# gnns4hri/3D_multi_pose_estimator

Hardware: AMD Instinct MI355X
Metric: frames/sec (5-view Panoptic, 4 persons) at 1/2/4/8 GPUs; MPJPE vs ref (higher is better)
Workload: dtype f32

## Files before the change

3d_multi_pose_estimator_amd/csrc/api.hip:

```cpp
#include <cmath>
#include <cstdarg>
#include <new>
#include <cstdio>
#include <cstdlib>
#include <cstring>

#include "mpe_internal.h"

using namespace mpe;

namespace {

int fail(mpe_ctx *ctx, int code, const char *fmt, ...) {
    char buf[512];
    va_list ap;
    va_start(ap, fmt);
    vsnprintf(buf, sizeof buf, fmt, ap);
    va_end(ap);
    if (ctx) ctx->err = buf;
    return code;
}

#define HIPCHK(ctx, expr)                                                                     \
    do {                                                                                      \
// ... 361 lines not shown
    const int V = ctx->cfg.n_cameras, J = ctx->cfg.n_joints, npj = ctx->cfg.numbers_per_joint;
    if (ctx->mlp[0].in_dim != V * J * npj)
        return fail(ctx, MPE_ERR_INVALID, "MLP input width %d != V*J*numbers_per_joint = %d", ctx->mlp[0].in_dim,
                    V * J * npj);
    int widest = 0;
    for (int l = 0; l < ctx->mlp_layers; ++l) {
        if (l > 0 && ctx->mlp[l].in_dim != ctx->mlp[l - 1].out_dim)
            return fail(ctx, MPE_ERR_INVALID, "MLP layer %d input width mismatch", l);
        widest = widest > ctx->mlp[l].out_dim ? widest : ctx->mlp[l].out_dim;
    }
    ctx->mlp_ld_in = round_up(ctx->mlp[0].in_dim, 128);
    ctx->mlp_ld_hidden = round_up(widest, 128);
    const size_t rows = (size_t)ctx->cfg.max_frames * ctx->cfg.max_persons_per_frame;
    int rc;
    if ((rc = dev_alloc(ctx, &ctx->mlp_rows, rows * ctx->mlp_ld_in))) return rc;
    for (int i = 0; i < 2; ++i)
        if ((rc = dev_alloc(ctx, &ctx->mlp_act[i], rows * ctx->mlp_ld_hidden))) return rc;
    ctx->mlp_ws_ready = true;
    return MPE_OK;
}

enum GatInput {
    GAT_IN_IMPLICIT,
    GAT_IN_DENSE0,
    GAT_IN_ACT
};

int gat_layer_linear(mpe_ctx *ctx, hipStream_t s, const mpe_batch *b, int l, GatInput in, AggArgs *a, int *n_rows_ft2) {
    GatLayer &g = ctx->gat[l];
    const int V = ctx->cfg.n_cameras, J = ctx->cfg.n_joints;
    const int n_nodes = b->n_heads + b->n_edge_nodes;
    const bool red = ctx->gat_reduced;
    const bool half_rows = red || ctx->gat_attn_fp16;
    const int ld_ft = half_rows ? 2 * ctx->act_ld : ctx->act_ld;
    int rc;
    const AttnCoef coef{g.attn_l, g.attn_r, ctx->a12, g.heads, g.out_dim};
    const bool no_epi = getenv("MPE_NO_COEF_EPILOGUE") != nullptr;
    const AttnCoef *cp = no_epi ? nullptr : &coef;
    bool done = false;
    if (in == GAT_IN_DENSE0) {
        if ((rc = gat_linear(ctx, s, ctx->xdense, ctx->feat_ld, g.fc1, ctx->hdense, ctx->feat_ld, n_nodes, nullptr,
                             true, ctx->gat_alpha, false)))
            return rc;
        if ((rc = gat_linear(ctx, s, ctx->hdense, ctx->feat_ld, g.fc2, ctx->act[2], ld_ft, n_nodes, nullptr, false,
                             0.f, half_rows, nullptr, nullptr, -1.0, cp, &done)))
            return rc;
        a->ft2 = ctx->act[2];
        *n_rows_ft2 = n_nodes;
    } else if (in == GAT_IN_IMPLICIT) {
        if (ctx->l0_grouped && !red && linear_uses_tile_kernel(b->n_heads, g.in_dim)) {
            GemmProf gp(ctx, s, 2.0 * b->n_heads * (double)g.in_dim * (J * 10), 0, 0);
            HIPCHK(ctx, launch_linear_grouped(s, ctx->xc, ctx->l0_ld, ctx->l0_w, ctx->l0_ld,
                                              (long)weight_rows(g.in_dim) * ctx->l0_ld, ctx->l0_b, ctx->h0, ctx->feat_ld,
                                              b->n_heads, ctx->cam_count, V, ctx->cam_list, ctx->cfg.max_heads, g.in_dim,
                                              ctx->l0_ld, true, ctx->gat_alpha, ctx->gat_acc64));
        } else if (ctx->l0_grouped) {
            const double flop_each = 2.0 * b->n_heads * (double)g.in_dim * (J * 10) / V;
            for (int c = 0; c < V; ++c)
                if ((rc = gat_linear(ctx, s, ctx->xc, ctx->l0_ld, ctx->l0_fc1[c], ctx->h0, ctx->feat_ld, b->n_heads,
                                     ctx->cam_count + c, true, ctx->gat_alpha, false,
                                     ctx->cam_list + (size_t)c * ctx->cfg.max_heads,
                                     ctx->cam_list + (size_t)c * ctx->cfg.max_heads, flop_each)))
                    return rc;
        } else if ((rc = gat_linear(ctx, s, ctx->x0, ctx->feat_ld, g.fc1, ctx->h0, ctx->feat_ld, b->n_heads, nullptr,
                                    true, ctx->gat_alpha, false)))
            return rc;
        if ((rc = gat_linear(ctx, s, ctx->h0, ctx->feat_ld, g.fc2, ctx->act[1], ld_ft, b->n_heads, nullptr, false,
                             0.f, half_rows, nullptr, nullptr, -1.0, cp, &done)))
            return rc;
        a->ft2 = ctx->act[1];
        *n_rows_ft2 = b->n_heads;
        a->en_const_ft2 = ctx->en0_ft2;
        a->en_const_a = ctx->en0_a;
    } else {
        if ((rc = gat_linear(ctx, s, ctx->act[0], ctx->act_ld, g.fc1, ctx->act[1], ctx->act_ld, n_nodes, nullptr,
                             true, ctx->gat_alpha, false)))
            return rc;
        if ((rc = gat_linear(ctx, s, ctx->act[1], ctx->act_ld, g.fc2, ctx->act[2], ld_ft, n_nodes, nullptr, false,
                             0.f, half_rows, nullptr, nullptr, -1.0, cp, &done)))
            return rc;
        a->ft2 = ctx->act[2];
        *n_rows_ft2 = n_nodes;
    }
    if (!done && cp && g.out_dim == 40 && !half_rows && ctx->gat_split && !red) {
        HIPCHK(ctx, launch_attn_coef(s, a->ft2, ld_ft, *n_rows_ft2, g.heads, g.out_dim, g.attn_l, g.attn_r, ctx->a12, 0));
        done = true;
    }
    a->a12_ready = done ? 1 : 0;
    return MPE_OK;
}

AggArgs gat_agg_args(const mpe_ctx *ctx, int l) {
    const GatLayer &g = ctx->gat[l];
    AggArgs a{};
    a.heads = g.heads;
    a.out_dim = g.out_dim;
    a.alpha = ctx->gat_alpha;
    a.out_slope = ctx->gat_hidden_slope;
    const bool half_rows = ctx->gat_reduced || ctx->gat_attn_fp16;
    a.ft_half = half_rows ? 1 : 0;
    a.ld = half_rows ? 2 * ctx->act_ld : ctx->act_ld;
    a.a12 = ctx->a12;
    return a;
}

void agg_scores_out(const mpe_ctx *ctx, AggArgs *a, float *d_scores_en, float *d_scores_heads) {
    a->out_mode = ctx->gat_out_mode;
    a->score_mode = 1;
    a->out = d_scores_en;
    a->out_heads = d_scores_heads;
    a->ld_out = 1;
}

int gat_attention(mpe_ctx *ctx, hipStream_t s, const mpe_batch *b, int l, const AggArgs &a, int n_rows_ft2) {
    const GatLayer &g = ctx->gat[l];
    HIPCHK(ctx, launch_gat_attention(s, *b, ctx->cfg.n_cameras, ctx->cfg.max_heads_per_frame, ctx->node_off,
                                     ctx->head_frame, ctx->en_frame, ctx->en_pair, g.attn_l, g.attn_r, ctx->a12, a,
                                     n_rows_ft2, ctx->head_src, explicit_deg_cap(ctx->cfg.max_heads_per_frame), ctx->x_m_cap));
    return MPE_OK;
}

int gat_topology(mpe_ctx *ctx, hipStream_t s, const mpe_batch *b) {
    if (b->d_en_pair && (size_t)b->n_frames * ctx->cfg.max_heads_per_frame * explicit_deg_cap(ctx->cfg.max_heads_per_frame) > ctx->head_src_cap)
        return fail(ctx, MPE_ERR_CAPACITY, "in-edge table too small for %d frames with explicit edge-node lists", b->n_frames);
    HIPCHK(ctx, launch_topology(s, *b, ctx->cfg.n_cameras, ctx->node_off, ctx->head_frame, ctx->en_frame, ctx->en_pair,
                                ctx->cfg.max_heads_per_frame, ctx->d_status, ctx->head_src,
                                explicit_deg_cap(ctx->cfg.max_heads_per_frame), ctx->x_m_cap));
    return MPE_OK;
}

constexpr int LAT_MAX_FRAMES = 16;
constexpr int LAT_MAX_NODES = 16384;

bool lat_gat_ok(mpe_ctx *ctx, const mpe_batch *b, bool dense_in) {
    if (!latency_path_on() || dense_in || b->d_en_pair || b->n_frames > LAT_MAX_FRAMES) return false;
    if (b->n_heads + b->n_edge_nodes > LAT_MAX_NODES || b->n_heads <= 0) return false;
    if (!ctx->gat_split || ctx->gat_acc64 || ctx->gat_reduced || ctx->gat_attn_fp16 || !ctx->l0_grouped) return false;
    if (getenv("MPE_NO_COEF_EPILOGUE") || getenv("MPE_GAT_ACC64_MINK") || getenv("MPE_SKINNY_WAVES") || getenv("MPE_GEMM_NARROW")) return false;
    if (!lat_l0a_available(ctx->cfg.n_joints, ctx->l0_ld)) return false;
    const GatLayer &g0 = ctx->gat[0];
    if (g0.out_dim != 40 || g0.in_dim <= 512) return false;
    for (int l = 1; l < ctx->gat_layers; ++l) {
        const GatLayer &g = ctx->gat[l];
        if (!lat_gemm_available(g.fc1.ldw, g.in_dim, false, 0) || !lat_gemm_available(g.fc2.ldw, g.heads * g.out_dim, true, g.out_dim)) return false;
        if (g.in_dim > 512) return false;
    }
    const size_t shm = (size_t)2 * ((size_t)16 * (ctx->cfg.max_heads_per_frame + 1) + (ctx->cfg.max_heads_per_frame + 1) + 1 +
                                    (size_t)(ctx->cfg.n_cameras + 1) * (ctx->cfg.n_cameras + 1)) * sizeof(float);
    return shm <= 40 * 1024;
}

int ensure_lat_workspace(mpe_ctx *ctx) {
    if (ctx->gat_pl[0]) return MPE_OK;
    ctx->lat_rows = ctx->max_nodes < LAT_MAX_NODES ? ctx->max_nodes : LAT_MAX_NODES;
    ctx->gat_pl_plane = (size_t)ctx->lat_rows * ctx->act_ld;
    int rc;
    for (int i = 0; i < 2; ++i)
        if ((rc = dev_alloc(ctx, &ctx->gat_pl[i], 3 * ctx->gat_pl_plane))) return rc;
    return MPE_OK;
}

struct LatTail {
    bool deferred = false;
    const float *ft2 = nullptr;
    int ld = 0;
    float alpha = 0.f, out_slope = 0.f;
    int out_mode = 0;
// ... 1053 lines not shown
```

3d_multi_pose_estimator_amd/csrc/gat.hip:

```cpp
#include <cstdlib>

#include "mpe_internal.h"
#include "sb_common.h"

namespace mpe {

__device__ __forceinline__ void topology_body(int f, int n_frames, int V, const int32_t *__restrict__ head_off,
                                              const int32_t *__restrict__ en_off, const int32_t *__restrict__ slot_n,
                                              int32_t *__restrict__ node_off, int32_t *__restrict__ head_frame,
                                              int32_t *__restrict__ en_frame, int32_t *__restrict__ en_pair, int hmax,
                                              int32_t *__restrict__ status) {
    __shared__ int s_n[MPE_MAX_CAMERAS], s_start[MPE_MAX_CAMERAS];
    const int h0 = head_off[f], H = head_off[f + 1] - h0;
    const int e0 = en_off[f], M = en_off[f + 1] - e0;
    if (threadIdx.x == 0) {
        int acc = 0;
        for (int s = 0; s < V; ++s) {
            s_n[s] = slot_n[f * V + s];
            s_start[s] = acc;
            acc += s_n[s];
        }
        node_off[f] = h0 + e0;
        if (H > hmax && status) atomicOr(status, 1);
        if (f == n_frames - 1) node_off[n_frames] = head_off[n_frames] + en_off[n_frames];
// ... 973 lines not shown
            }
            mx = wave_max(mx);
            float sum = 0.f;
            for (int e = lane; e < deg; e += 64) {
                const float ex = expf(w[e] - mx);
                w[e] = ex;
                sum = sum + ex;
            }
            sum = wave_sum(sum);
            for (int e = lane; e < deg; e += 64) w[e] = w[e] / sum;
        }
    }
    __syncthreads();

    const int per_row = hd / VEC;
    for (int i = t; i < AGG_ROWS * per_row; i += blockDim.x) {
        const int r = i / per_row, c = (i - r * per_row) * VEC;
        const int dg = s_deg[r];
        if (dg == 0) continue;
        const int ff = s_f[r], vv = s_v[r], HH = s_H[r];
        const int hh = c / a.out_dim;
        const int32_t nbb = node_off[ff], hbb = head_off[ff];
        const float *w = s_w + ((size_t)r * heads + hh) * max_deg;
        const int *src = s_src + r * max_deg;
        float acc[VEC];
        weighted_sum8<VEC>(
            dg,
            [&](int e, float *fv) {
                const int u = src[e];
                if (l0 && u >= HH) ld_ftv<VEC>(a.en_const_ft2, (size_t)c, 0, fv);
                else ld_ftv<VEC>(a.ft2, (size_t)((l0 ? hbb : nbb) + u) * a.ld + c, a.ft_half, fv);
            },
            [&](int e) { return w[e]; }, acc);
        if (a.score_mode) {
            a.out_heads[(size_t)hbb + vv] = agg_activate(acc[0], a.out_mode, a.out_slope);
        } else {
            float o[VEC];
#pragma unroll
            for (int k = 0; k < VEC; ++k) o[k] = agg_activate(acc[k], a.out_mode, a.out_slope);
            agg_store_row<VEC>(a, (size_t)(nbb + vv), c, o);
        }
    }
}

template <int VEC>
__global__ __launch_bounds__(256) void k_aggregate_heads(
    int n_heads, int V, int max_deg, const int32_t *__restrict__ head_off, const int32_t *__restrict__ en_off,
    const int32_t *__restrict__ slot_n, const int32_t *__restrict__ node_off,
    const int32_t *__restrict__ head_frame, AggArgs a, const uint16_t *__restrict__ head_src, int src_stride, int hmax) {
    extern __shared__ float s_dyn[];
    aggregate_heads_body<VEC>(blockIdx.x, s_dyn, n_heads, V, max_deg, head_off, en_off, slot_n, node_off, head_frame, a, head_src, src_stride, hmax);
}

constexpr int LAT_EN_ROWS = 2;
template <int VEC>
__global__ __launch_bounds__(256) void k_lat_attention(
    int n_en_wgs, int n_en, int n_heads, int V, int max_deg, const int32_t *__restrict__ head_off, const int32_t *__restrict__ en_off,
    const int32_t *__restrict__ slot_n, const int32_t *__restrict__ node_off, const int32_t *__restrict__ head_frame,
    const int32_t *__restrict__ en_frame, const int32_t *__restrict__ en_pair, AggArgs a, const uint16_t *__restrict__ head_src,
    int src_stride, int hmax) {
    extern __shared__ float s_dyn[];
    if ((int)blockIdx.x < n_en_wgs) {
        aggregate_en_body<VEC, LAT_EN_ROWS>(blockIdx.x, n_en, head_off, en_off, node_off, en_frame, en_pair, a, hmax);
    } else if (!a.score_mode || a.out_heads) {
        aggregate_heads_body<VEC>(blockIdx.x - n_en_wgs, s_dyn, n_heads, V, max_deg, head_off, en_off, slot_n, node_off, head_frame, a, head_src,
                                  src_stride, hmax);
    }
}

__host__ __device__ inline size_t fused_tables_floats(int hmax, int max_deg, int V, int n_cap, int m_cap) {
    const size_t deg = (size_t)max_deg;
    const size_t n = 2 * (size_t)n_cap + 2 * hmax * deg + (size_t)m_cap * 4 + (V + 1) + (size_t)V * V + MPE_MAX_CAMERAS + hmax;
    return (n + 255) & ~(size_t)255;
}

__device__ __forceinline__ void lds_barrier() {
    __builtin_amdgcn_fence(__ATOMIC_RELEASE, "workgroup", "local");
    __builtin_amdgcn_s_barrier();
    __builtin_amdgcn_fence(__ATOMIC_ACQUIRE, "workgroup", "local");
}

__device__ __forceinline__ void lds_barrier_raw() { asm volatile("s_waitcnt lgkmcnt(0)\n\ts_barrier" ::: "memory"); }

constexpr int FUSED_PIECES = 8;

#ifdef MPE_FUSED_CLOCK
__device__ unsigned int g_fused_stamp[16384][4];
#define FUSED_STAMP(SLOT)                                                                \
    do {                                                                                 \
        if (threadIdx.x == 0) {                                                          \
            const unsigned long long now_ = __builtin_amdgcn_s_memrealtime();            \
            g_fused_stamp[blockIdx.x & 16383][SLOT] = (unsigned int)(now_ - fused_t_);   \
            fused_t_ = now_;                                                             \
        }                                                                                \
    } while (0)
#else
#define FUSED_STAMP(SLOT) do { } while (0)
#endif

template <int VEC, int G>
__global__ __launch_bounds__(256) void k_gat_fused(int V, int max_deg, int hmax, int n_cap, int m_cap,
                                                   const int32_t *__restrict__ head_off,
                                                   const int32_t *__restrict__ en_off,
                                                   const int32_t *__restrict__ slot_n,
                                                   const int32_t *__restrict__ node_off,
                                                   const int32_t *__restrict__ en_pair,
                                                   const float *__restrict__ attn_l,
                                                   const float *__restrict__ attn_r, AggArgs a, int overlap,
                                                   const uint16_t *__restrict__ head_src) {
#pragma clang fp contract(off)
    typedef float vecf __attribute__((ext_vector_type(VEC)));
    extern __shared__ __attribute__((aligned(1024))) float s_dyn[];
    const int bid = blockIdx.x, nwg = gridDim.x;
#ifdef MPE_FUSED_CLOCK
    unsigned long long fused_t_ = __builtin_amdgcn_s_memrealtime();
#endif
    const int xcd = bid & 7, xq = nwg >> 3, xr = nwg & 7;
    const int vid = (xcd < xr ? xcd * (xq + 1) : xr * (xq + 1) + (xcd - xr) * xq) + (bid >> 3);
    const int f = vid / a.heads, hh = vid - f * a.heads;
    const int D = a.out_dim;
    const int hb = head_off[f], H = head_off[f + 1] - hb;
    const int eb = en_off[f], M = en_off[f + 1] - eb;
    const int N = H + M, nb = node_off[f];
    if (M <= 0) return;
    if (H > hmax || N > n_cap || M > m_cap) {
        if (a.score_mode)
            for (int m = threadIdx.x; m < M; m += blockDim.x) a.out[(size_t)eb + m] = 0.f;
        return;
    }
    const int Dp = D;
    float *s_a1 = s_dyn;
    float *s_a2 = s_a1 + n_cap;
    float *s_wh = s_a2 + n_cap;
    int *s_src = reinterpret_cast<int *>(s_wh + (size_t)hmax * max_deg);
    int *s_pair = s_src + (size_t)hmax * max_deg;
    float *s_wen = reinterpret_cast<float *>(s_pair + m_cap);
    FrameTopo tp;
    tp.start = reinterpret_cast<int *>(s_wen + (size_t)m_cap * 3);
    tp.base = tp.start + V + 1;
    int *s_sn = tp.base + V * V;
    int *s_deg = s_sn + MPE_MAX_CAMERAS;
    float *s_ft = s_dyn + fused_tables_floats(hmax, max_deg, V, n_cap, m_cap);
    const int t = threadIdx.x, lane = t & 63, wave = t >> 6;
    const bool l0 = a.en_const_ft2 != nullptr;
    const int c0 = hh * D;
    const int DV = D / VEC;
    const int32_t *sn = slot_n + (size_t)f * V;

    if (VEC == 4 && (overlap & 1)) {
        const int total = N * DV;
        const size_t row0 = (size_t)(l0 ? hb : nb);
        const int tn = t < N ? t : N - 1, tm = t < M ? t : M - 1;
        const int n_src2 = hmax * max_deg / 2;
        const int ts = t < n_src2 ? t : n_src2 - 1;
        const float *pr_ = (l0 && tn >= H) ? a.en_const_a : a.a12 + (row0 + tn) * 32;
        const float *p1 = pr_ + hh, *p2 = pr_ + 16 + hh;
        const int32_t *pe = en_pair + 2 * (size_t)(eb + tm);
        const uint32_t *ps = reinterpret_cast<const uint32_t *>(head_src + (size_t)f * hmax * max_deg) + ts;
        const float *src[FUSED_PIECES];
#pragma unroll
        for (int u = 0; u < FUSED_PIECES; ++u) {
            int c = wave * 64 + u * 256 + lane;
            c = c < total ? c : total - 1;
            const int node = c / DV, d = (c - node * DV) * 4;
            src[u] = (l0 && node >= H) ? a.en_const_ft2 + (c0 + d) : a.ft2 + (row0 + node) * a.ld + c0 + d;
        }
        const unsigned m0v = __builtin_amdgcn_readfirstlane(
            (unsigned)(size_t)(__attribute__((address_space(3))) float *)s_ft + (unsigned)(wave * 64) * 16u);
        float r1, r2;
        int e1, e2;
        uint32_t sv;
        unsigned m0_keep;
        static_assert(FUSED_PIECES == 8, "the asm block below issues eight pieces and waits for vmcnt(8)");
        asm volatile(
            "s_mov_b32 %[keep], m0\n\t"
            "global_load_dword %[r1], %[p1], off\n\t"
            "global_load_dword %[r2], %[p2], off\n\t"
            "global_load_dword %[e1], %[pe], off\n\t"
            "global_load_dword %[e2], %[pe], off offset:4\n\t"
            "global_load_dword %[sv], %[ps], off\n\t"
            "s_mov_b32 m0, %[m0v]\n\t"
            "s_nop 0\n\t"
            "global_load_lds_dwordx4 %[s0], off\n\t"
            "s_add_u32 m0, m0, 0x1000\n\t"
            "s_nop 0\n\t"
            "global_load_lds_dwordx4 %[s1], off\n\t"
            "s_add_u32 m0, m0, 0x1000\n\t"
            "s_nop 0\n\t"
            "global_load_lds_dwordx4 %[s2], off\n\t"
            "s_add_u32 m0, m0, 0x1000\n\t"
            "s_nop 0\n\t"
            "global_load_lds_dwordx4 %[s3], off\n\t"
            "s_add_u32 m0, m0, 0x1000\n\t"
            "s_nop 0\n\t"
            "global_load_lds_dwordx4 %[s4], off\n\t"
            "s_add_u32 m0, m0, 0x1000\n\t"
            "s_nop 0\n\t"
            "global_load_lds_dwordx4 %[s5], off\n\t"
            "s_add_u32 m0, m0, 0x1000\n\t"
            "s_nop 0\n\t"
            "global_load_lds_dwordx4 %[s6], off\n\t"
            "s_add_u32 m0, m0, 0x1000\n\t"
            "s_nop 0\n\t"
            "global_load_lds_dwordx4 %[s7], off\n\t"
            "s_mov_b32 m0, %[keep]\n\t"
            "s_waitcnt vmcnt(8)"
            : [r1] "=&v"(r1), [r2] "=&v"(r2), [e1] "=&v"(e1), [e2] "=&v"(e2), [sv] "=&v"(sv), [keep] "=&s"(m0_keep)
            : [p1] "v"(p1), [p2] "v"(p2), [pe] "v"(pe), [ps] "v"(ps), [m0v] "s"(m0v), [s0] "v"(src[0]), [s1] "v"(src[1]),
              [s2] "v"(src[2]), [s3] "v"(src[3]), [s4] "v"(src[4]), [s5] "v"(src[5]), [s6] "v"(src[6]), [s7] "v"(src[7])
            : "memory", "scc");
        if (t < N) {
            s_a1[t] = r1;
            s_a2[t] = r2;
        }
        if (t < M) s_pair[t] = (e1 << 16) | e2;
        if (t < n_src2) {
            const int lo = sv & 0xFFFF, hi = sv >> 16;
            s_src[2 * t] = lo == 0xFFFF ? -1 : lo;
            s_src[2 * t + 1] = hi == 0xFFFF ? -1 : hi;
        }
        FUSED_STAMP(0);
        lds_barrier_raw();
    } else {
    if (VEC == 4 && !a.ft_half) {
        const int total = N * DV;
        for (int c0_ = wave * 64; c0_ < total; c0_ += 256) {
            int c = c0_ + lane;
            c = c < total ? c : total - 1;
            const int node = c / DV, d = (c - node * DV) * 4;
            const float *src = (l0 && node >= H) ? a.en_const_ft2 + (c0 + d)
                                                  : a.ft2 + (size_t)((l0 ? hb : nb) + node) * a.ld + c0 + d;
            __builtin_amdgcn_global_load_lds((const __attribute__((address_space(1))) void *)src,
                                             (__attribute__((address_space(3))) void *)(s_ft + (size_t)c0_ * 4), 16, 0, 0);
        }
    } else if (!a.ft_half) {
        const int total = N * D;
        for (int c0_ = wave * 64; c0_ < total; c0_ += 256) {
            int c = c0_ + lane;
            c = c < total ? c : total - 1;
            const int node = c / D, d = c - node * D;
            const float *src = (l0 && node >= H) ? a.en_const_ft2 + (c0 + d)
                                                  : a.ft2 + (size_t)((l0 ? hb : nb) + node) * a.ld + c0 + d;
            __builtin_amdgcn_global_load_lds((const __attribute__((address_space(1))) void *)src,
                                             (__attribute__((address_space(3))) void *)(s_ft + (size_t)c0_), 4, 0, 0);
        }
    } else {
        const int total = N * DV;
        for (int i0 = t; i0 < total; i0 += 4 * blockDim.x) {
            float v[4][VEC];
#pragma unroll
            for (int u = 0; u < 4; ++u) {
                int i = i0 + u * blockDim.x;
                i = i < total ? i : total - 1;
                const int node = i / DV, d = (i - node * DV) * VEC;
                if (l0 && node >= H) ld_ftv<VEC>(a.en_const_ft2, (size_t)(c0 + d), 0, v[u]);
                else ld_ftv<VEC>(a.ft2, (size_t)((l0 ? hb : nb) + node) * a.ld + c0 + d, a.ft_half, v[u]);
            }
#pragma unroll
            for (int u = 0; u < 4; ++u) {
                const int i = i0 + u * blockDim.x;
                if (i < total) {
                    const int node = i / DV, d = (i - node * DV) * VEC;
                    vecf o;
#pragma unroll
                    for (int k = 0; k < VEC; ++k) o[k] = v[u][k];
                    *reinterpret_cast<vecf *>(s_ft + node * Dp + d) = o;
                }
            }
        }
    }
    if (a.a12_ready) {
        for (int node = t; node < N; node += blockDim.x) {
            const float *r = (l0 && node >= H) ? a.en_const_a : a.a12 + (size_t)((l0 ? hb : nb) + node) * 32;
            s_a1[node] = r[hh];
            s_a2[node] = r[16 + hh];
        }
    }
    for (int m = t; m < M; m += blockDim.x)
        s_pair[m] = (en_pair[2 * (size_t)(eb + m)] << 16) | en_pair[2 * (size_t)(eb + m) + 1];
    if (head_src) {
        const uint16_t *tab = head_src + (size_t)f * hmax * max_deg;
        for (int i = t; i < H * max_deg; i += blockDim.x) {
            const int u = tab[i];
            s_src[i] = u == 0xFFFF ? -1 : u;
        }
        __syncthreads();
    } else {
        if (t < V) s_sn[t] = sn[t];
        __syncthreads();
        build_topo(tp, s_sn, V, H, t, blockDim.x);
        __syncthreads();
        for (int i = t; i < H * max_deg; i += blockDim.x) {
            const int h = i / max_deg, e = i - h * max_deg;
            const int sl = slot_of_head(tp, V, h);
            s_src[i] = e < 1 + H - s_sn[sl] ? head_in_edge(tp, s_sn, V, h, sl, e) : -1;
        }
        __syncthreads();
    }
    }
    if (!a.a12_ready) {
        for (int node = t; node < N; node += blockDim.x) {
            const float *fv = s_ft + node * Dp;
            float x1 = 0.f, x2 = 0.f;
            if (D == 40) {
                coef40([&](int d) { return fv[d]; }, attn_l + c0, attn_r + c0, hh & 1, x1, x2);
            } else {
                for (int d = 0; d < D; ++d) {
                    x1 = __builtin_fmaf(fv[d], attn_l[c0 + d], x1);
                    x2 = __builtin_fmaf(fv[d], attn_r[c0 + d], x2);
                }
            }
            s_a1[node] = x1;
            s_a2[node] = x2;
        }
        __syncthreads();
    }
    for (int m = t; m < M; m += blockDim.x) {
        const int pr = s_pair[m];
        const int h1 = pr >> 16, h2 = pr & 0xFFFF, x = H + m;
        const float a2v = s_a2[x];
        float e1 = s_a1[h1] + a2v, e2 = s_a1[h2] + a2v, e3 = s_a1[x] + a2v;
        e1 = e1 > 0.f ? e1 : e1 * a.alpha;
        e2 = e2 > 0.f ? e2 : e2 * a.alpha;
        e3 = e3 > 0.f ? e3 : e3 * a.alpha;
        const float mx = fmaxf(fmaxf(e1, e2), e3);
        const float x1 = expf(e1 - mx), x2 = expf(e2 - mx), x3 = expf(e3 - mx);
        const float sum = (x1 + x2) + x3;
        s_wen[m * 3 + 0] = x1 / sum;
        s_wen[m * 3 + 1] = x2 / sum;
        s_wen[m * 3 + 2] = x3 / sum;
    }
    if (!a.score_mode || a.out_heads) {
        const int gl = t & (G - 1);
        for (int h = t / G; h < H; h += 256 / G) {
            float *w = s_wh + h * max_deg;
            const int *src = s_src + h * max_deg;
            const float a2v = s_a2[h];
            float mx = -INFINITY;
            int deg = 0;
            for (int e = gl; e < max_deg; e += G) {
                const int u = src[e];
                if (u >= 0) {
                    float x = s_a1[u] + a2v;
                    x = x > 0.f ? x : x * a.alpha;
                    w[e] = x;
                    mx = fmaxf(mx, x);
                    deg = e + 1;
                }
            }
            mx = group_max<G>(mx);
            deg = (int)group_max<G>((float)deg);
            float sum = 0.f;
            for (int e = gl; e < deg; e += G) {
                const float ex = expf(w[e] - mx);
                w[e] = ex;
                sum = sum + ex;
            }
            sum = group_sum<G>(sum);
            for (int e = gl; e < deg; e += G) w[e] = w[e] / sum;
            if (gl == 0) s_deg[h] = deg;
        }
    }
    FUSED_STAMP(1);
    __syncthreads();
    FUSED_STAMP(2);
    const int first = (a.score_mode && !a.out_heads) ? H : 0;
    if (VEC == 4 && !a.score_mode && (DV & 1) == 0 && !(overlap & 2)) {
        const int DV2 = DV / 2;
        const int n_head_items = H * DV, n_items = n_head_items + M * DV2;
        for (int i = t; i < n_items; i += blockDim.x) {
            if (i >= n_head_items) {
                const int j = i - n_head_items;
                const int m = j / DV2, d = (j - m * DV2) * 8;
                const int node = H + m;
                const int pr = s_pair[m];
                const int h1 = pr >> 16, h2 = pr & 0xFFFF;
                const float w1 = s_wen[m * 3 + 0], w2 = s_wen[m * 3 + 1], w3 = s_wen[m * 3 + 2];
                const float *p1 = s_ft + h1 * Dp + d, *p2 = s_ft + h2 * Dp + d, *p3 = s_ft + node * Dp + d;
                float *dst = a.out + (size_t)(nb + node) * a.ld_out + c0 + d;
#pragma unroll
                for (int g = 0; g < 2; ++g) {
                    const vecf f1 = *reinterpret_cast<const vecf *>(p1 + 4 * g);
                    const vecf f2 = *reinterpret_cast<const vecf *>(p2 + 4 * g);
                    const vecf f3 = *reinterpret_cast<const vecf *>(p3 + 4 * g);
                    vecf o;
#pragma unroll
                    for (int k = 0; k < VEC; ++k) {
                        float acc = f1[k] * w1;
                        acc = acc + f2[k] * w2;
                        acc = acc + f3[k] * w3;
                        o[k] = agg_activate(acc, a.out_mode, a.out_slope);
                    }
                    *reinterpret_cast<vecf *>(dst + 4 * g) = o;
                }
            } else {
                const int node = i / DV, d = (i - node * DV) * VEC;
                const int deg = s_deg[node];
                const int *src = s_src + node * max_deg;
                const float *w = s_wh + node * max_deg;
                float acc[VEC];
                weighted_sum8<VEC>(
                    deg,
                    [&](int e, float *fv) {
                        const vecf x = *reinterpret_cast<const vecf *>(s_ft + src[e] * Dp + d);
#pragma unroll
                        for (int k = 0; k < VEC; ++k) fv[k] = x[k];
                    },
                    [&](int e) { return w[e]; }, acc);
                vecf o;
#pragma unroll
                for (int k = 0; k < VEC; ++k) o[k] = agg_activate(acc[k], a.out_mode, a.out_slope);
                *reinterpret_cast<vecf *>(a.out + (size_t)(nb + node) * a.ld_out + c0 + d) = o;
            }
        }
        FUSED_STAMP(3);
        return;
    }
    for (int i = first * DV + t; i < N * DV; i += blockDim.x) {
        const int node = i / DV, d = (i - node * DV) * VEC;
        vecf o;
        if (node >= H) {
            const int m = node - H;
            const int pr = s_pair[m];
            const int h1 = pr >> 16, h2 = pr & 0xFFFF;
            const float w1 = s_wen[m * 3 + 0], w2 = s_wen[m * 3 + 1], w3 = s_wen[m * 3 + 2];
            const vecf f1 = *reinterpret_cast<const vecf *>(s_ft + h1 * Dp + d);
            const vecf f2 = *reinterpret_cast<const vecf *>(s_ft + h2 * Dp + d);
            const vecf f3 = *reinterpret_cast<const vecf *>(s_ft + node * Dp + d);
#pragma unroll
            for (int k = 0; k < VEC; ++k) {
                float acc = f1[k] * w1;
                acc = acc + f2[k] * w2;
                acc = acc + f3[k] * w3;
                o[k] = agg_activate(acc, a.out_mode, a.out_slope);
            }
        } else {
            const int deg = s_deg[node];
            const int *src = s_src + node * max_deg;
            const float *w = s_wh + node * max_deg;
            float acc[VEC];
            weighted_sum8<VEC>(
                deg,
                [&](int e, float *fv) {
                    const vecf x = *reinterpret_cast<const vecf *>(s_ft + src[e] * Dp + d);
#pragma unroll
                    for (int k = 0; k < VEC; ++k) fv[k] = x[k];
                },
                [&](int e) { return w[e]; }, acc);
#pragma unroll
            for (int k = 0; k < VEC; ++k) o[k] = agg_activate(acc[k], a.out_mode, a.out_slope);
        }
        if (a.score_mode) {
            if (node >= H) a.out[(size_t)eb + (node - H)] = o[0];
            else a.out_heads[(size_t)hb + node] = o[0];
        } else {
            *reinterpret_cast<vecf *>(a.out + (size_t)(nb + node) * a.ld_out + c0 + d) = o;
        }
    }
    FUSED_STAMP(3);
}

#ifdef MPE_FUSED_CLOCK
}
extern "C" int mpe_debug_fused_stamps(unsigned int *out, int clear) {
    if (hipMemcpyFromSymbol(out, HIP_SYMBOL(mpe::g_fused_stamp), sizeof(mpe::g_fused_stamp)) != hipSuccess) return -1;
    if (clear) {
        void *p = nullptr;
        if (hipGetSymbolAddress(&p, HIP_SYMBOL(mpe::g_fused_stamp)) != hipSuccess || hipMemset(p, 0, sizeof(mpe::g_fused_stamp)) != hipSuccess) return -1;
    }
    return 0;
}
namespace mpe {
#endif

static size_t fused_lds_bytes(int hmax, int V, int out_dim, int *n_cap, int *m_cap, int *max_deg, int x_deg_cap, int x_m_cap) {
    const int mc = x_m_cap > 0 ? x_m_cap : hmax * hmax * (V - 1) / (2 * V) + 1;
    const int nc = hmax + mc;
    const int deg = x_m_cap > 0 ? x_deg_cap : hmax + 1;
    const int Dp = out_dim;
    size_t image = (size_t)nc * Dp + 256;
    if (out_dim % 4 == 0 && image < (size_t)FUSED_PIECES * 1024)
        image = (size_t)FUSED_PIECES * 1024;
    const size_t bytes = (fused_tables_floats(hmax, deg, V, nc, mc) + image) * sizeof(float);
    *n_cap = nc;
    *m_cap = mc;
    *max_deg = deg;
    return bytes;
}

static int agg_vec(const AggArgs &a) {
    if (!a.score_mode && a.ld % 4 == 0 && a.ld_out % 4 == 0) {
        if (a.out_dim % 4 == 0) return 4;
        if (a.out_dim % 2 == 0) return 2;
    }
    return 1;
}

static bool half_vec8() {
    static const bool v = !(getenv("MPE_HALF_VEC") && atoi(getenv("MPE_HALF_VEC")) == 4);
    return v;
}

constexpr size_t FUSED_LDS_LIMIT = 160 * 1024;

hipError_t launch_gat_attention(hipStream_t s, const mpe_batch &b, int V, int max_heads_per_frame,
                                const int32_t *node_off, const int32_t *head_frame, const int32_t *en_frame,
                                const int32_t *en_pair, const float *attn_l, const float *attn_r, float *a12,
                                const AggArgs &a, int n_rows_ft2, const uint16_t *head_src, int x_deg_cap, int x_m_cap) {
    int n_cap, m_cap, max_deg;
    const bool xpl = b.d_en_pair != nullptr;
    if (xpl && (!head_src || x_m_cap <= 0)) return hipErrorInvalidValue;
    if (!xpl) x_deg_cap = x_m_cap = 0;
    if (!xpl && getenv("MPE_NO_HEAD_SRC_TABLE")) head_src = nullptr;
    const size_t shm = fused_lds_bytes(max_heads_per_frame, V, a.out_dim, &n_cap, &m_cap, &max_deg, x_deg_cap, x_m_cap);
    const bool no_fuse = getenv("MPE_NO_FUSED_ATTENTION") != nullptr;
    if (shm <= FUSED_LDS_LIMIT && !no_fuse && b.n_frames > 0) {
        const int vec = agg_vec(a);
        const int grp = max_deg <= 32 ? 16 : max_deg <= 64 ? 32 : 64;
        if (!xpl && !head_src_entries(max_heads_per_frame, V)) head_src = nullptr;
        const int overlap = ((!xpl && vec == 4 && a.a12_ready && !a.ft_half && n_cap <= 256 && m_cap <= 256 && head_src &&
                              max_heads_per_frame * (max_heads_per_frame + 1) <= 512 &&
                              n_cap * (a.out_dim / 4) <= FUSED_PIECES * 256 && !getenv("MPE_FUSED_NO_OVERLAP")) ? 1 : 0) |
                            (getenv("MPE_FUSED_NO_OVERLAP") ? 2 : 0);
        const void *fn = nullptr;
#define MPE_FUSED(V_, G_)                                                                                     \
    do {                                                                                                      \
        fn = reinterpret_cast<const void *>(k_gat_fused<V_, G_>);                                             \
        if (shm > 64 * 1024) {                                                                                \
            hipError_t e_ = hipFuncSetAttribute(fn, hipFuncAttributeMaxDynamicSharedMemorySize, (int)FUSED_LDS_LIMIT); \
            if (e_ != hipSuccess) return e_;                                                                  \
        }                                                                                                     \
        hipLaunchKernelGGL((k_gat_fused<V_, G_>), dim3(b.n_frames * a.heads), dim3(256), shm, s, V,            \
                           max_deg, max_heads_per_frame, n_cap, m_cap, b.d_frame_head_off, b.d_frame_en_off, b.d_slot_n, \
                           node_off, en_pair, attn_l, attn_r, a, overlap, head_src);                          \
    } while (0)
#define MPE_FUSED_G(V_)                     \
    do {                                    \
        if (grp == 16) MPE_FUSED(V_, 16);   \
        else if (grp == 32) MPE_FUSED(V_, 32); \
        else MPE_FUSED(V_, 64);             \
    } while (0)
        if (vec == 4) MPE_FUSED_G(4);
        else if (vec == 2) MPE_FUSED_G(2);
        else MPE_FUSED_G(1);
#undef MPE_FUSED_G
#undef MPE_FUSED
        return hipGetLastError();
    }
    AggArgs a2 = a;
    a2.a12 = a12;
    if (!a.a12_ready) {
        hipError_t e = launch_attn_coef(s, a.ft2, a.ld, n_rows_ft2, a.heads, a.out_dim, attn_l, attn_r, a12, a.ft_half);
        if (e != hipSuccess) return e;
        a2.a12_ready = 1;
    }
    return launch_aggregate(s, b, V, max_heads_per_frame, node_off, head_frame, en_frame, en_pair, a2, head_src, x_deg_cap);
}

hipError_t launch_lat_attention(hipStream_t s, const mpe_batch &b, int V, int max_heads_per_frame, const int32_t *node_off,
                                const int32_t *head_frame, const int32_t *en_frame, const int32_t *en_pair, const AggArgs &a,
                                const uint16_t *head_src) {
    if (b.d_en_pair || a.ft_half || (!a.a12_ready && (!a.attn_l || !a.attn_r))) return hipErrorInvalidValue;
    const int vec = agg_vec(a);
    if (!head_src_entries(max_heads_per_frame, V)) head_src = nullptr;
    const int n_en_wgs = (b.n_edge_nodes + LAT_EN_ROWS - 1) / LAT_EN_ROWS;
    const bool heads_on = b.n_heads > 0 && (!a.score_mode || a.out_heads);
    const int n_h_wgs = heads_on ? (b.n_heads + AGG_ROWS - 1) / AGG_ROWS : 0;
    if (n_en_wgs + n_h_wgs == 0) return hipSuccess;
    const int src_stride = max_heads_per_frame + 1;
    int max_deg = src_stride < 3 ? 3 : src_stride;
    const size_t shm = (size_t)AGG_ROWS * ((size_t)a.heads * max_deg + max_deg + (V + 1) + (size_t)V * V + 16) * sizeof(float);
    if (shm > 48 * 1024) return hipErrorInvalidValue;
    const int hd4 = (a.heads * a.out_dim + 3) / 4 * 4;
    (void)hd4;
#define MPE_LA(V_)                                                                                                              \
    hipLaunchKernelGGL(k_lat_attention<V_>, dim3(n_en_wgs + n_h_wgs), dim3(256), shm, s, n_en_wgs, b.n_edge_nodes, b.n_heads, V, max_deg, \
                       b.d_frame_head_off, b.d_frame_en_off, b.d_slot_n, node_off, head_frame, en_frame, en_pair, a, head_src, src_stride, \
                       max_heads_per_frame)
    if (vec == 4) MPE_LA(4);
    else if (vec == 2) MPE_LA(2);
    else MPE_LA(1);
#undef MPE_LA
    return hipGetLastError();
}

hipError_t launch_aggregate(hipStream_t s, const mpe_batch &b, int V, int max_heads_per_frame,
                            const int32_t *node_off, const int32_t *head_frame, const int32_t *en_frame,
                            const int32_t *en_pair, const AggArgs &a, const uint16_t *head_src, int x_deg_cap) {
    const int vec = agg_vec(a);
    const bool xpl = b.d_en_pair != nullptr;
    if (xpl && (!head_src || x_deg_cap <= 0)) return hipErrorInvalidValue;
    if (!xpl && !head_src_entries(max_heads_per_frame, V)) head_src = nullptr;
    if (b.n_edge_nodes > 0) {
        const unsigned blocks = (unsigned)((b.n_edge_nodes + EN_ROWS - 1) / EN_ROWS);
#define MPE_EN(V_)                                                                                      \
    hipLaunchKernelGGL(k_aggregate_en<V_>, dim3(blocks), dim3(256), 0, s, b.n_edge_nodes, b.d_frame_head_off, \
                       b.d_frame_en_off, node_off, en_frame, en_pair, a, max_heads_per_frame)
        const int hd4 = (a.heads * a.out_dim + 3) / 4 * 4;
        const bool wide = !a.score_mode && !a.ft_half && a.ld % 4 == 0 && a.ld_out % 4 == 0 && hd4 <= a.ld && hd4 <= a.ld_out &&
                          !a.en_const_ft2;
        if (vec == 4 && a.ft_half && a.out_dim % 8 == 0 && half_vec8()) MPE_EN(8);
        else if (vec == 4 || wide) MPE_EN(4);
        else if (vec == 2) MPE_EN(2);
        else MPE_EN(1);
#undef MPE_EN
        hipError_t e = hipGetLastError();
        if (e != hipSuccess) return e;
    }
    if (b.n_heads > 0 && (!a.score_mode || a.out_heads)) {
        const int src_stride = xpl ? x_deg_cap : max_heads_per_frame + 1;
        int max_deg = src_stride;
        if (max_deg < 3) max_deg = 3;
        const size_t shm = (size_t)AGG_ROWS * ((size_t)a.heads * max_deg + max_deg + (V + 1) + (size_t)V * V + 16) * sizeof(float);
        if (shm > 64 * 1024) {
            static PerDeviceFlag attr;
            if (!attr.test()) {
                hipError_t e = hipSuccess;
                const void *fns[4] = {reinterpret_cast<const void *>(k_aggregate_heads<8>), reinterpret_cast<const void *>(k_aggregate_heads<4>),
                                      reinterpret_cast<const void *>(k_aggregate_heads<2>), reinterpret_cast<const void *>(k_aggregate_heads<1>)};
                for (const void *fn : fns)
                    if (e == hipSuccess) e = hipFuncSetAttribute(fn, hipFuncAttributeMaxDynamicSharedMemorySize, (int)FUSED_LDS_LIMIT);
                if (e != hipSuccess) return e;
                attr.set();
            }
        }
        const int grid = (b.n_heads + AGG_ROWS - 1) / AGG_ROWS;
#define MPE_HEADS(V_)                                                                                   \
    hipLaunchKernelGGL(k_aggregate_heads<V_>, dim3(grid), dim3(256), shm, s, b.n_heads, V, max_deg,         \
                       b.d_frame_head_off, b.d_frame_en_off, b.d_slot_n, node_off, head_frame, a, head_src,       \
                       src_stride, max_heads_per_frame)
        if (vec == 4 && a.ft_half && a.out_dim % 8 == 0 && half_vec8()) MPE_HEADS(8);
        else if (vec == 4) MPE_HEADS(4);
        else if (vec == 2) MPE_HEADS(2);
        else MPE_HEADS(1);
#undef MPE_HEADS
    }
    return hipGetLastError();
}

}
```

Measured before the change: 267,600.

## Add compact layer-0 and wide-row variants of fused GAT attention kernel

Turns the fused GAT kernel into a templated body with two new forms. In the layer-0 compact form, all edge nodes share one constant feature row, so only H+1 rows are staged in LDS and attention coefficients for edge nodes come from precomputed constants. In the wide form for VEC==2, rows are padded to 4-float alignment so they can be staged with 16-byte global-to-LDS loads instead of 4-byte ones. Both aim to cut LDS footprint and staging traffic, at the cost of more template variants and offset bookkeeping. The layer-0 path now also recomputes attention coefficients in-kernel instead of using the precomputed overlap path.

```diff
diff --git a/3d_multi_pose_estimator_amd/csrc/api.hip b/3d_multi_pose_estimator_amd/csrc/api.hip
--- a/3d_multi_pose_estimator_amd/csrc/api.hip
+++ b/3d_multi_pose_estimator_amd/csrc/api.hip
@@ -467,7 +467,7 @@
         a->ft2 = ctx->act[2];
         *n_rows_ft2 = n_nodes;
     }
-    if (!done && cp && g.out_dim == 40 && !half_rows && ctx->gat_split && !red) {
+    if (!done && cp && g.out_dim == 40 && !half_rows && ctx->gat_split && !red && in != GAT_IN_IMPLICIT) {
         HIPCHK(ctx, launch_attn_coef(s, a->ft2, ld_ft, *n_rows_ft2, g.heads, g.out_dim, g.attn_l, g.attn_r, ctx->a12, 0));
         done = true;
     }
diff --git a/3d_multi_pose_estimator_amd/csrc/gat.hip b/3d_multi_pose_estimator_amd/csrc/gat.hip
--- a/3d_multi_pose_estimator_amd/csrc/gat.hip
+++ b/3d_multi_pose_estimator_amd/csrc/gat.hip
@@ -1079,6 +1079,8 @@
 
 __device__ __forceinline__ void lds_barrier_raw() { asm volatile("s_waitcnt lgkmcnt(0)\n\ts_barrier" ::: "memory"); }
 
+__host__ __device__ inline int fused_wide_dp(int D) { return (D + 2 + 3) / 4 * 4; }
+
 constexpr int FUSED_PIECES = 8;
 
 #ifdef MPE_FUSED_CLOCK
@@ -1095,16 +1097,16 @@
 #define FUSED_STAMP(SLOT) do { } while (0)
 #endif
 
-template <int VEC, int G>
-__global__ __launch_bounds__(256) void k_gat_fused(int V, int max_deg, int hmax, int n_cap, int m_cap,
-                                                   const int32_t *__restrict__ head_off,
-                                                   const int32_t *__restrict__ en_off,
-                                                   const int32_t *__restrict__ slot_n,
-                                                   const int32_t *__restrict__ node_off,
-                                                   const int32_t *__restrict__ en_pair,
-                                                   const float *__restrict__ attn_l,
-                                                   const float *__restrict__ attn_r, AggArgs a, int overlap,
-                                                   const uint16_t *__restrict__ head_src) {
+template <int VEC, int G, bool L0C>
+__device__ __forceinline__ void gat_fused_body(int V, int max_deg, int hmax, int n_cap, int m_cap,
+                                               const int32_t *__restrict__ head_off,
+                                               const int32_t *__restrict__ en_off,
+                                               const int32_t *__restrict__ slot_n,
+                                               const int32_t *__restrict__ node_off,
+                                               const int32_t *__restrict__ en_pair,
+                                               const float *__restrict__ attn_l,
+                                               const float *__restrict__ attn_r, const AggArgs &a, int overlap,
+                                               const uint16_t *__restrict__ head_src) {
 #pragma clang fp contract(off)
     typedef float vecf __attribute__((ext_vector_type(VEC)));
     extern __shared__ __attribute__((aligned(1024))) float s_dyn[];
@@ -1125,7 +1127,10 @@
             for (int m = threadIdx.x; m < M; m += blockDim.x) a.out[(size_t)eb + m] = 0.f;
         return;
     }
-    const int Dp = D;
+    const bool wide = VEC == 2 && (overlap & 4);
+    const int Dp = wide ? fused_wide_dp(D) : D;
+    const int fo = wide ? (hh * D) & 3 : 0;
+    const int NI = L0C ? H + 1 : N;
     float *s_a1 = s_dyn;
     float *s_a2 = s_a1 + n_cap;
     float *s_wh = s_a2 + n_cap;
@@ -1137,14 +1142,16 @@
     tp.base = tp.start + V + 1;
     int *s_sn = tp.base + V * V;
     int *s_deg = s_sn + MPE_MAX_CAMERAS;
-    float *s_ft = s_dyn + fused_tables_floats(hmax, max_deg, V, n_cap, m_cap);
+    float *s_ft0 = s_dyn + fused_tables_floats(hmax, max_deg, V, n_cap, m_cap);
+    const float *s_ft = s_ft0 + fo;
     const int t = threadIdx.x, lane = t & 63, wave = t >> 6;
-    const bool l0 = a.en_const_ft2 != nullptr;
+    const bool l0 = L0C || a.en_const_ft2 != nullptr;
+    auto row_of = [&](int node) { return L0C ? (node < H ? node : H) : node; };
     const int c0 = hh * D;
     const int DV = D / VEC;
     const int32_t *sn = slot_n + (size_t)f * V;
 
-    if (VEC == 4 && (overlap & 1)) {
+    if (VEC == 4 && !L0C && (overlap & 1)) {
         const int total = N * DV;
         const size_t row0 = (size_t)(l0 ? hb : nb);
         const int tn = t < N ? t : N - 1, tm = t < M ? t : M - 1;
@@ -1163,7 +1170,7 @@
             src[u] = (l0 && node >= H) ? a.en_const_ft2 + (c0 + d) : a.ft2 + (row0 + node) * a.ld + c0 + d;
         }
         const unsigned m0v = __builtin_amdgcn_readfirstlane(
-            (unsigned)(size_t)(__attribute__((address_space(3))) float *)s_ft + (unsigned)(wave * 64) * 16u);
+            (unsigned)(size_t)(__attribute__((address_space(3))) float *)s_ft0 + (unsigned)(wave * 64) * 16u);
         float r1, r2;
         int e1, e2;
         uint32_t sv;
@@ -1220,7 +1227,7 @@
         lds_barrier_raw();
     } else {
     if (VEC == 4 && !a.ft_half) {
-        const int total = N * DV;
+        const int total = NI * DV;
         for (int c0_ = wave * 64; c0_ < total; c0_ += 256) {
             int c = c0_ + lane;
             c = c < total ? c : total - 1;
@@ -1228,7 +1235,17 @@
             const float *src = (l0 && node >= H) ? a.en_const_ft2 + (c0 + d)
                                                   : a.ft2 + (size_t)((l0 ? hb : nb) + node) * a.ld + c0 + d;
             __builtin_amdgcn_global_load_lds((const __attribute__((address_space(1))) void *)src,
-                                             (__attribute__((address_space(3))) void *)(s_ft + (size_t)c0_ * 4), 16, 0, 0);
+                                             (__attribute__((address_space(3))) void *)(s_ft0 + (size_t)c0_ * 4), 16, 0, 0);
+        }
+    } else if (wide) {
+        const int CH = Dp / 4, total = N * CH;
+        for (int c0_ = wave * 64; c0_ < total; c0_ += 256) {
+            int c = c0_ + lane;
+            c = c < total ? c : total - 1;
+            const int node = c / CH, d = (c - node * CH) * 4;
+            const float *src = a.ft2 + (size_t)(nb + node) * a.ld + (c0 - fo) + d;
+            __builtin_amdgcn_global_load_lds((const __attribute__((address_space(1))) void *)src,
+                                             (__attribute__((address_space(3))) void *)(s_ft0 + (size_t)c0_ * 4), 16, 0, 0);
         }
     } else if (!a.ft_half) {
         const int total = N * D;
@@ -1239,7 +1256,7 @@
             const float *src = (l0 && node >= H) ? a.en_const_ft2 + (c0 + d)
                                                   : a.ft2 + (size_t)((l0 ? hb : nb) + node) * a.ld + c0 + d;
             __builtin_amdgcn_global_load_lds((const __attribute__((address_space(1))) void *)src,
-                                             (__attribute__((address_space(3))) void *)(s_ft + (size_t)c0_), 4, 0, 0);
+                                             (__attribute__((address_space(3))) void *)(s_ft0 + (size_t)c0_), 4, 0, 0);
         }
     } else {
         const int total = N * DV;
@@ -1261,7 +1278,7 @@
                     vecf o;
 #pragma unroll
                     for (int k = 0; k < VEC; ++k) o[k] = v[u][k];
-                    *reinterpret_cast<vecf *>(s_ft + node * Dp + d) = o;
+                    *reinterpret_cast<vecf *>(s_ft0 + node * Dp + d) = o;
                 }
             }
         }
@@ -1297,6 +1314,11 @@
     }
     if (!a.a12_ready) {
         for (int node = t; node < N; node += blockDim.x) {
+            if (L0C && node >= H) {
+                s_a1[node] = a.en_const_a[hh];
+                s_a2[node] = a.en_const_a[16 + hh];
+                continue;
+            }
             const float *fv = s_ft + node * Dp;
             float x1 = 0.f, x2 = 0.f;
             if (D == 40) {
@@ -1373,7 +1395,7 @@
                 const int pr = s_pair[m];
                 const int h1 = pr >> 16, h2 = pr & 0xFFFF;
                 const float w1 = s_wen[m * 3 + 0], w2 = s_wen[m * 3 + 1], w3 = s_wen[m * 3 + 2];
-                const float *p1 = s_ft + h1 * Dp + d, *p2 = s_ft + h2 * Dp + d, *p3 = s_ft + node * Dp + d;
+                const float *p1 = s_ft + h1 * Dp + d, *p2 = s_ft + h2 * Dp + d, *p3 = s_ft + row_of(node) * Dp + d;
                 float *dst = a.out + (size_t)(nb + node) * a.ld_out + c0 + d;
 #pragma unroll
                 for (int g = 0; g < 2; ++g) {
@@ -1399,7 +1421,7 @@
                 weighted_sum8<VEC>(
                     deg,
                     [&](int e, float *fv) {
-                        const vecf x = *reinterpret_cast<const vecf *>(s_ft + src[e] * Dp + d);
+                        const vecf x = *reinterpret_cast<const vecf *>(s_ft + row_of(src[e]) * Dp + d);
 #pragma unroll
                         for (int k = 0; k < VEC; ++k) fv[k] = x[k];
                     },
@@ -1423,7 +1445,7 @@
             const float w1 = s_wen[m * 3 + 0], w2 = s_wen[m * 3 + 1], w3 = s_wen[m * 3 + 2];
             const vecf f1 = *reinterpret_cast<const vecf *>(s_ft + h1 * Dp + d);
             const vecf f2 = *reinterpret_cast<const vecf *>(s_ft + h2 * Dp + d);
-            const vecf f3 = *reinterpret_cast<const vecf *>(s_ft + node * Dp + d);
+            const vecf f3 = *reinterpret_cast<const vecf *>(s_ft + row_of(node) * Dp + d);
 #pragma unroll
             for (int k = 0; k < VEC; ++k) {
                 float acc = f1[k] * w1;
@@ -1439,7 +1461,7 @@
             weighted_sum8<VEC>(
                 deg,
                 [&](int e, float *fv) {
-                    const vecf x = *reinterpret_cast<const vecf *>(s_ft + src[e] * Dp + d);
+                    const vecf x = *reinterpret_cast<const vecf *>(s_ft + row_of(src[e]) * Dp + d);
 #pragma unroll
                     for (int k = 0; k < VEC; ++k) fv[k] = x[k];
                 },
@@ -1457,6 +1479,34 @@
     FUSED_STAMP(3);
 }
 
+template <int VEC, int G>
+__global__ __launch_bounds__(256) void k_gat_fused(int V, int max_deg, int hmax, int n_cap, int m_cap,
+                                                   const int32_t *__restrict__ head_off,
+                                                   const int32_t *__restrict__ en_off,
+                                                   const int32_t *__restrict__ slot_n,
+                                                   const int32_t *__restrict__ node_off,
+                                                   const int32_t *__restrict__ en_pair,
+                                                   const float *__restrict__ attn_l,
+                                                   const float *__restrict__ attn_r, AggArgs a, int overlap,
+                                                   const uint16_t *__restrict__ head_src) {
+    gat_fused_body<VEC, G, false>(V, max_deg, hmax, n_cap, m_cap, head_off, en_off, slot_n, node_off, en_pair, attn_l, attn_r, a,
+                                  overlap, head_src);
+}
+
+template <int G>
+__global__ __launch_bounds__(256) void k_gat_fused_l0(int V, int max_deg, int hmax, int n_cap, int m_cap,
+                                                      const int32_t *__restrict__ head_off,
+                                                      const int32_t *__restrict__ en_off,
+                                                      const int32_t *__restrict__ slot_n,
+                                                      const int32_t *__restrict__ node_off,
+                                                      const int32_t *__restrict__ en_pair,
+                                                      const float *__restrict__ attn_l,
+                                                      const float *__restrict__ attn_r, AggArgs a, int overlap,
+                                                      const uint16_t *__restrict__ head_src) {
+    gat_fused_body<4, G, true>(V, max_deg, hmax, n_cap, m_cap, head_off, en_off, slot_n, node_off, en_pair, attn_l, attn_r, a,
+                               overlap, head_src);
+}
+
 #ifdef MPE_FUSED_CLOCK
 }
 extern "C" int mpe_debug_fused_stamps(unsigned int *out, int clear) {
@@ -1470,13 +1520,14 @@
 namespace mpe {
 #endif
 
-static size_t fused_lds_bytes(int hmax, int V, int out_dim, int *n_cap, int *m_cap, int *max_deg, int x_deg_cap, int x_m_cap) {
+enum FusedForm { FUSED_FULL = 0, FUSED_L0_COMPACT = 1, FUSED_WIDE = 2 };
+size_t fused_lds_bytes(int hmax, int V, int out_dim, int *n_cap, int *m_cap, int *max_deg, int x_deg_cap, int x_m_cap, int form) {
     const int mc = x_m_cap > 0 ? x_m_cap : hmax * hmax * (V - 1) / (2 * V) + 1;
     const int nc = hmax + mc;
     const int deg = x_m_cap > 0 ? x_deg_cap : hmax + 1;
-    const int Dp = out_dim;
-    size_t image = (size_t)nc * Dp + 256;
-    if (out_dim % 4 == 0 && image < (size_t)FUSED_PIECES * 1024)
+    const int Dp = form == FUSED_WIDE ? fused_wide_dp(out_dim) : out_dim;
+    size_t image = (size_t)(form == FUSED_L0_COMPACT ? hmax + 1 : nc) * Dp + 256;
+    if (form == FUSED_FULL && out_dim % 4 == 0 && image < (size_t)FUSED_PIECES * 1024)
         image = (size_t)FUSED_PIECES * 1024;
     const size_t bytes = (fused_tables_floats(hmax, deg, V, nc, mc) + image) * sizeof(float);
     *n_cap = nc;
@@ -1509,16 +1560,22 @@
     if (xpl && (!head_src || x_m_cap <= 0)) return hipErrorInvalidValue;
     if (!xpl) x_deg_cap = x_m_cap = 0;
     if (!xpl && getenv("MPE_NO_HEAD_SRC_TABLE")) head_src = nullptr;
-    const size_t shm = fused_lds_bytes(max_heads_per_frame, V, a.out_dim, &n_cap, &m_cap, &max_deg, x_deg_cap, x_m_cap);
+    const int vec = agg_vec(a);
+    const bool l0c = !xpl && a.en_const_ft2 && a.en_const_a && vec == 4 && !a.ft_half && attn_l && attn_r;
+    const bool wide = !l0c && !a.en_const_ft2 && vec == 2 && !a.ft_half && (a.heads * a.out_dim + 3) / 4 * 4 <= a.ld &&
+                      fused_lds_bytes(max_heads_per_frame, V, a.out_dim, &n_cap, &m_cap, &max_deg, x_deg_cap, x_m_cap, FUSED_WIDE) <= FUSED_LDS_LIMIT;
+    const size_t shm_full = fused_lds_bytes(max_heads_per_frame, V, a.out_dim, &n_cap, &m_cap, &max_deg, x_deg_cap, x_m_cap, FUSED_FULL);
+    const size_t shm = !(l0c || wide) ? shm_full
+                                      : fused_lds_bytes(max_heads_per_frame, V, a.out_dim, &n_cap, &m_cap, &max_deg, x_deg_cap, x_m_cap,
+                                                        l0c ? FUSED_L0_COMPACT : FUSED_WIDE);
     const bool no_fuse = getenv("MPE_NO_FUSED_ATTENTION") != nullptr;
-    if (shm <= FUSED_LDS_LIMIT && !no_fuse && b.n_frames > 0) {
-        const int vec = agg_vec(a);
+    if (shm_full <= FUSED_LDS_LIMIT && !no_fuse && b.n_frames > 0) {
         const int grp = max_deg <= 32 ? 16 : max_deg <= 64 ? 32 : 64;
         if (!xpl && !head_src_entries(max_heads_per_frame, V)) head_src = nullptr;
         const int overlap = ((!xpl && vec == 4 && a.a12_ready && !a.ft_half && n_cap <= 256 && m_cap <= 256 && head_src &&
                               max_heads_per_frame * (max_heads_per_frame + 1) <= 512 &&
                               n_cap * (a.out_dim / 4) <= FUSED_PIECES * 256 && !getenv("MPE_FUSED_NO_OVERLAP")) ? 1 : 0) |
-                            (getenv("MPE_FUSED_NO_OVERLAP") ? 2 : 0);
+                            (getenv("MPE_FUSED_NO_OVERLAP") ? 2 : 0) | (wide ? 4 : 0);
         const void *fn = nullptr;
 #define MPE_FUSED(V_, G_)                                                                                     \
     do {                                                                                                      \
@@ -1537,7 +1594,25 @@
         else if (grp == 32) MPE_FUSED(V_, 32); \
         else MPE_FUSED(V_, 64);             \
     } while (0)
-        if (vec == 4) MPE_FUSED_G(4);
+        if (l0c) {
+            AggArgs a0 = a;
+            a0.a12_ready = 0;
+#define MPE_FUSED_L0(G_)                                                                                      \
+    do {                                                                                                      \
+        if (shm > 64 * 1024) {                       \
+            hipError_t e_ = hipFuncSetAttribute(reinterpret_cast<const void *>(k_gat_fused_l0<G_>),           \
+                                                hipFuncAttributeMaxDynamicSharedMemorySize, (int)FUSED_LDS_LIMIT); \
+            if (e_ != hipSuccess) return e_;                                                                  \
+        }                                                                                                     \
+        hipLaunchKernelGGL((k_gat_fused_l0<G_>), dim3(b.n_frames * a.heads), dim3(256), shm, s, V, max_deg,   \
+                           max_heads_per_frame, n_cap, m_cap, b.d_frame_head_off, b.d_frame_en_off, b.d_slot_n, \
+                           node_off, en_pair, attn_l, attn_r, a0, overlap & 2, head_src);                     \
+    } while (0)
+            if (grp == 16) MPE_FUSED_L0(16);
+            else if (grp == 32) MPE_FUSED_L0(32);
+            else MPE_FUSED_L0(64);
+#undef MPE_FUSED_L0
+        } else if (vec == 4) MPE_FUSED_G(4);
         else if (vec == 2) MPE_FUSED_G(2);
         else MPE_FUSED_G(1);
 #undef MPE_FUSED_G
@@ -1636,3 +1711,9 @@
 }
 
 }
+
+extern "C" size_t mpe_debug_fused_lds_bytes(int hmax, int V, int out_dim, int layer0) {
+    int n_cap, m_cap, max_deg;
+    const int form = layer0 ? mpe::FUSED_L0_COMPACT : (out_dim % 4 != 0 && out_dim % 2 == 0) ? mpe::FUSED_WIDE : mpe::FUSED_FULL;
+    return mpe::fused_lds_bytes(hmax, V, out_dim, &n_cap, &m_cap, &max_deg, 0, 0, form);
+}
```

New measurement: 262,400. 0.98x the previous value.
